# dylandreimerink/gobpfld

Measured on AMD Instinct MI355X. Metric: Mpkt/s device-resident XDP-emulator verdicts, 64B and 1500B batches, higher is better.
Workload: dtype int64

## Files before the change

### gobpfld_amd/csrc/xe_jit.cpp

```cpp
#ifndef XE_HOSTSIM
#include <hip/hip_runtime_api.h>
#include <hip/hiprtc.h>
#endif

#include <algorithm>
#include <array>
#include <atomic>
#include <chrono>
#include <climits>
#include <cstdint>
#include <cstdio>
#include <cstdlib>
#include <cstring>
#include <fstream>
#include <future>
#include <map>
#include <memory>
#include <set>
#include <mutex>
#include <sstream>
#include <string>
#include <vector>

#include <unistd.h>
// ... 1780 lines not shown
  if (buf && buflen) {
    const size_t c = s.size() < buflen - 1 ? s.size() : buflen - 1;
    memcpy(buf, s.data(), c);
    buf[c] = 0;
  }
  return s.size();
}

#ifndef XE_HOSTSIM
extern "C" int xe_jit_occupancy(void* fn, uint32_t nmaps) {
  int nb = 0;
  if (hipModuleOccupancyMaxActiveBlocksPerMultiprocessor(&nb, (hipFunction_t)fn, 256, (nmaps + 1) * sizeof(XeDevMap)) != hipSuccess) return 0;
  return nb;
}

extern "C" int xe_jit_launch(void* fn, const XeParams* P, uint32_t blocks, uint32_t threads, hipStream_t s) {
  XeParams p = *P;
  void* args[] = {&p};
  return hipModuleLaunchKernel((hipFunction_t)fn, blocks, 1, 1, threads, 1, 1, unsigned((p.nmaps + 1) * sizeof(XeDevMap)), s, args,
                               nullptr) == hipSuccess ? 0 : -1;
}

extern "C" int xe_jit_compile_check(const XeUop* prog, size_t n, char* buf, size_t buflen) {
  std::vector<XeUop> p(prog, prog + n);
  std::string err;
  std::vector<char> code = compile(generate_vm({std::vector<XeUop>(), p}, 1, demo_geom(), XE_JV_PLAIN, nullptr, nullptr), "gfx950", err);
  if (buf && buflen) {
    size_t c = err.size() < buflen - 1 ? err.size() : buflen - 1;
    memcpy(buf, err.data(), c);
    buf[c] = 0;
  }
  return code.empty() ? -1 : 0;
}

extern "C" int xe_jit_compile_check_keyed(const XeUop* prog, size_t n, char* buf, size_t buflen) {
// ... 47 lines not shown
```

### gobpfld_amd/csrc/xe_kernel.hip

```cpp
#include "xe_interp.h"
#include "xe_kernels.h"

#include <hipcub/device/device_radix_sort.hpp>
#include <hipcub/device/device_scan.hpp>

extern "C" __global__ void __launch_bounds__(256) xe_interp_kernel(XeParams P) {
  __shared__ __attribute__((aligned(16))) uint8_t hdr_lds[XE_HDR_LDS_BYTES];
  __shared__ XePend pend_lds[4];
  extern __shared__ __attribute__((aligned(16))) uint8_t xe_dyn_lds[];
  XeLane L;
  L.hdrbuf = (XE_LP(uint8_t))(hdr_lds + (threadIdx.x >> 6) * XE_HDR_WAVE_BYTES);
  const int lane = xe_lane();
  stage_maps(L, P, (XE_LP(XeDevMap))xe_dyn_lds);
  wave_state_init(L, P, (blockIdx.x * blockDim.x + threadIdx.x) >> 6, &pend_lds[threadIdx.x >> 6]);
  if (P.mode == XE_MODE_SEQUENTIAL) {
    if (blockIdx.x != 0 || threadIdx.x >= 64) return;
    seq_packets(L, P, [&](uint32_t i, bool valid) { run_staged(L, P, i, valid); }, [](bool) {});
  } else if (P.mode == XE_MODE_CHAIN) {
    chain_packets(L, P, blockIdx.x * blockDim.x + threadIdx.x, gridDim.x * blockDim.x,
                  [&](uint32_t i, bool valid) { run_staged(L, P, i, valid); });
  } else {
    const uint32_t wave = (blockIdx.x * blockDim.x + threadIdx.x) >> 6;
    const uint32_t nwaves = (gridDim.x * blockDim.x) >> 6;
    parallel_packets(L, P, wave, nwaves, [&](uint32_t i, bool valid) { run_staged(L, P, i, valid); });
// ... 49 lines not shown
  uint32_t nseg;
  unsigned long long* zero;
  uint64_t zero_words;
};
extern "C" __global__ void xe_prologue_kernel(XeProlog A) {
  const uint64_t tid = blockIdx.x * uint64_t(blockDim.x) + threadIdx.x, nth = uint64_t(gridDim.x) * blockDim.x;
  for (uint64_t i = tid; i < A.zero_words; i += nth) A.zero[i] = 0;
  for (uint32_t g = 0; g < A.nseg; g++)
    for (uint64_t i = tid; i < A.words[g]; i += nth) A.dst[g][i] = A.src[g][i];
}

extern "C" __global__ void __launch_bounds__(1024) xe_tail_kernel(XeTailArgs A) {
  __shared__ unsigned long long orw[257];
  const uint32_t t = threadIdx.x, nt = blockDim.x;
  for (uint32_t w = t; w <= 256; w += nt) orw[w] = 0;
  const bool poisoned = *(volatile uint32_t*)A.poison != 0;
  __syncthreads();
  for (uint32_t i = t; i < A.aux_words; i += nt) {
    const unsigned long long v = A.aux[i];
    if (v) A.aux[i] = 0;
    A.host_aux[i] = v;
    if (i == 0) orw[256] = v;
    else if (i >= 16 && v) atomicOr(&orw[(i - 16) % A.rep_words], v);
  }
  __syncthreads();
  if (t == 0) {
    const bool replay = !poisoned && xe_replay_decision(uint32_t(orw[256]), orw, A.rep_words, A.nmaps, A.mode);
    A.host_aux[XE_AUX_DECISION] = replay ? 1ull : 0ull;
    if (replay) *A.poison = 1u;
  }
  if (poisoned) return;
  for (uint32_t f = 0; f < A.ntail; f++) {
    const XeTailMap& T = A.tail[f];
    for (uint64_t i = t; i < T.words; i += nt) {
      unsigned long long r[16];
#pragma unroll
      for (uint32_t k = 0; k < 16; k++) r[k] = k < T.nrep ? T.rep[k * T.stride_words + i] : 0ull;
      unsigned long long s = 0;
#pragma unroll
      for (uint32_t k = 0; k < 16; k++) {
        s += r[k];
        if (r[k]) T.rep[k * T.stride_words + i] = 0;
      }
      const unsigned long long v = T.vals[i] + s;
      if (s) T.vals[i] = v;
      T.snap[i] = v;
    }
  }
}
extern "C" int xe_launch_tail(const XeTailArgs* A, hipStream_t s) {
  if (A->rep_words > 256) return -1;
  hipLaunchKernelGGL(xe_tail_kernel, dim3(1), dim3(1024), 0, s, *A);
  return hipGetLastError() == hipSuccess ? 0 : -1;
}

__global__ void xe_desc_split_kernel(const xe_desc* d, uint32_t n, uint64_t umem_len, unsigned long long* key,
                                     uint32_t* len) {
  for (uint64_t i = blockIdx.x * uint64_t(blockDim.x) + threadIdx.x; i < n; i += uint64_t(gridDim.x) * blockDim.x) {
    const uint64_t a = d[i].addr;
    uint32_t l = d[i].len;
    if (a > umem_len || uint64_t(l) > umem_len - a) l = 0;
    key[i] = l ? a : ~0ull;
    len[i] = l;
  }
}
__global__ void xe_desc_overlap_kernel(const unsigned long long* key, const uint32_t* len, uint32_t n, uint32_t* flag) {
  for (uint64_t i = blockIdx.x * uint64_t(blockDim.x) + threadIdx.x; i + 1 < n; i += uint64_t(gridDim.x) * blockDim.x)
// ... 232 lines not shown

extern "C" int xe_launch_keyed_esort(const XeKeyed* K, void* scratch, size_t* bytes, hipStream_t s) {
  size_t tmp = 0;
  if (hipcub::DeviceRadixSort::SortPairs(nullptr, tmp, (const unsigned long long*)nullptr, (unsigned long long*)nullptr,
                                         (const uint32_t*)nullptr, (uint32_t*)nullptr, int(K->dcap), 0, 64, s) != hipSuccess)
    return -1;
  if (!scratch) {
    *bytes = tmp;
    return 0;
  }
  if (*bytes < tmp) return -1;
  return hipcub::DeviceRadixSort::SortPairs(scratch, tmp, (const unsigned long long*)K->ekey, (unsigned long long*)K->ekey2,
                                            K->eval, K->eval2, int(K->dcap), 0, 64, s) == hipSuccess ? 0 : -1;
}

extern "C" int xe_launch_interp(const XeParams* P, uint32_t blocks, uint32_t threads, hipStream_t s) {
  hipLaunchKernelGGL(xe_interp_kernel, dim3(blocks), dim3(threads), (P->nmaps + 1) * sizeof(XeDevMap), s, *P);
  return hipGetLastError() == hipSuccess ? 0 : -1;
}
extern "C" int xe_interp_occupancy(uint32_t nmaps) {
  int nb = 0;
  if (hipOccupancyMaxActiveBlocksPerMultiprocessor(&nb, xe_interp_kernel, 256, (nmaps + 1) * sizeof(XeDevMap)) != hipSuccess) return 0;
  return nb;
}
template <class T, class C = T>
static int launch_delta_t(const void* cur, const void* snap, void* out, uint64_t n, hipStream_t s) {
  uint32_t blocks = uint32_t(n / 256 + 1);
  if (blocks > 4096) blocks = 4096;
  hipLaunchKernelGGL((xe_delta_kernel<T, C>), dim3(blocks), dim3(256), 0, s, (const T*)cur, (const T*)snap, (C*)out, n);
  return hipGetLastError() == hipSuccess ? 0 : -1;
}
template <class T, class C = T>
// ... 70 lines not shown
```

### gobpfld_amd/csrc/xe_kernels.h

```cpp
#ifndef XE_KERNELS_H_
#define XE_KERNELS_H_

#include "xe_internal.h"

#ifndef XE_HOSTSIM
#include <hip/hip_runtime_api.h>
#endif

extern "C" {

int xe_jit_may_write_entries(const XeUop* prog, size_t n);
size_t xe_jit_source_for(const XeUop* const* progs, const uint32_t* lens, uint32_t nprogs, int32_t entry,
                         const XeDevMap* maps, uint32_t nmaps, int variant, char* buf, size_t buflen);

#ifndef XE_HOSTSIM
void* xe_jit_get(const XeUop* const* progs, const uint32_t* lens, uint32_t nprogs, int32_t entry, int device,
                 const XeDevMap* maps, uint32_t nmaps, bool* cyclic, bool* general, const char** err, int variant,
                 uint64_t* maxpath);
int xe_jit_launch(void* fn, const XeParams* P, uint32_t blocks, uint32_t threads, hipStream_t s);
int xe_jit_occupancy(void* fn, uint32_t nmaps);

int xe_launch_interp(const XeParams* P, uint32_t blocks, uint32_t threads, hipStream_t s);
int xe_interp_occupancy(uint32_t nmaps);
int xe_launch_delta(const void* cur, const void* snap, void* out, uint64_t bytes, uint32_t lane, hipStream_t s);
int xe_launch_apply_delta(void* cur, const void* snap, const void* delta, uint64_t bytes, uint32_t lane, hipStream_t s);
int xe_launch_delta_sum(void* acc, const void* in, uint64_t bytes, uint32_t lane, hipStream_t s);
int xe_launch_rep_fold(void* vals, void* rep, uint64_t stride_words, uint32_t nrep, uint64_t nwords, const void* recs,
                       uint32_t rwords, uint32_t vsize, uint32_t cap, const void* lim, hipStream_t s);
int xe_launch_prologue(const void* const* src, void* const* dst, const uint64_t* words, uint32_t nseg, void* zero,
                       uint64_t zero_words, hipStream_t s);
int xe_launch_tail(const XeTailArgs* A, hipStream_t s);
int xe_launch_desc_overlap(const void* desc, uint32_t n, uint64_t umem_len, void* scratch, size_t* scratch_bytes,
                           uint32_t* flag, hipStream_t s);
int xe_launch_keyed(const XeKeyed* K, const XeDevMap* maps, uint8_t* skip, uint32_t step, uint32_t items, hipStream_t s);
int xe_launch_keyed_sort(const XeKeyed* K, uint32_t n, uint32_t end_bit, void* scratch, size_t* bytes, hipStream_t s);
int xe_launch_keyed_esort(const XeKeyed* K, void* scratch, size_t* bytes, hipStream_t s);
int xe_launch_keyed_scan(const XeKeyed* K, uint32_t n, void* scratch, size_t* bytes, hipStream_t s);
int xe_launch_append(const XeAppendArgs* A, uint32_t end_bit, void* scratch, size_t* bytes, hipStream_t s);
int xe_launch_pop(const uint32_t* src, uint32_t* dst, uint32_t n, uint32_t mode, uint32_t arg, XePopSlots sl, uint32_t* flag,
                  hipStream_t s);
int xe_launch_lru_relink(uint64_t* tag, uint32_t pool, uint32_t cnt, uint32_t* link, uint64_t* hdr, void* scratch,
                         size_t* bytes, int renumber, hipStream_t s);
int xe_launch_lru_tag_fold(uint64_t* tag, uint64_t* rep, uint32_t pool, uint32_t r, const uint64_t* hdr, hipStream_t s);
int xe_launch_lru_log(const uint64_t* tag, uint32_t pool, const uint32_t* order, const uint64_t* hdr, uint64_t* log,
                      hipStream_t s);
#endif
// ... 14 lines not shown
```

### gobpfld_amd/csrc/xe_runtime.cpp

```cpp
#include "xe_internal.h"
#include "xe_mapops.h"

#include <algorithm>
#include <map>
#include <chrono>
#include <cstdio>
#include <cstdlib>
#include <cstring>
#include <string>
#include <array>
#include <thread>
#include <vector>

#ifdef XE_HOSTSIM
#define XE_SEQ_PEEK 1
#include "xe_interp.h"
typedef void* xe_stream_t;
#else
#include <hip/hip_runtime_api.h>
typedef hipStream_t xe_stream_t;
#endif
#include "xe_kernels.h"

#define XE_FRAME_SIZE 256

namespace {

#ifdef XE_HOSTSIM
#ifdef XE_HOSTSIM_POISON
int dev_alloc(void** p, size_t n) {
  n = n ? n : 8;
  *p = malloc(n);
  if (*p) memset(*p, 0xA5, n);
  return *p ? 0 : -1;
}
#else
int dev_alloc(void** p, size_t n) { *p = calloc(n ? n : 8, 1); return *p ? 0 : -1; }
#endif
void dev_free(void* p) { free(p); }
int h2d(void* d, const void* h, size_t n, xe_stream_t) { memcpy(d, h, n); return 0; }
int d2h(void* h, const void* d, size_t n, xe_stream_t) { memcpy(h, d, n); return 0; }
int d2d(void* d, const void* s, size_t n, xe_stream_t) { memmove(d, s, n); return 0; }
int dmemset(void* d, int v, size_t n, xe_stream_t) { memset(d, v, n); return 0; }
int dsync(xe_stream_t) { return 0; }
int launch_interp(const XeParams* P, uint32_t, uint32_t, xe_stream_t) {
  XeLane L;
#ifdef XE_HOSTSIM_POISON
  memset(static_cast<void*>(&L), 0, sizeof L);
#endif
  static thread_local uint8_t hdrbuf[XE_HDR_WAVE_BYTES + 16];
  L.hdrbuf = hdrbuf;
  XePend pend;
  stage_maps(L, *P, nullptr);
  wave_state_init(L, *P, 0, &pend);
  if (P->mode == XE_MODE_PARALLEL || P->mode == XE_MODE_SPEC) {
    parallel_packets(L, *P, 0, 1, [&](uint32_t i, bool valid) { run_staged(L, *P, i, valid); });
  } else if (P->mode == XE_MODE_CHAIN) {
    chain_packets(L, *P, 0, 1, [&](uint32_t i, bool valid) { run_staged(L, *P, i, valid); });
  } else {
    seq_packets(L, *P, [&](uint32_t i, bool valid) { run_staged(L, *P, i, valid); },
                [&](bool valid) { run_staged(L, *P, 0, valid, false); });
  }
  flush_wave_state(L, *P);
  return 0;
}
int launch_jit(void*, const XeParams* P, uint32_t b, uint32_t t, xe_stream_t s) { return launch_interp(P, b, t, s); }
template <class T, class C = T>
void lanes_sub(const void* a, const void* b, void* o, uint64_t n) {
  for (uint64_t i = 0; i < n; i++) ((C*)o)[i] = C(T(((const T*)a)[i] - ((const T*)b)[i]));
}
template <class T, class C = T>
void lanes_add(const void* snap, const void* d, void* o, uint64_t n) {
  for (uint64_t i = 0; i < n; i++) ((T*)o)[i] = T(((const T*)snap)[i] + T(((const C*)d)[i]));
}
template <class C>
void lanes_acc(void* acc, const void* in, uint64_t n) {
  for (uint64_t i = 0; i < n; i++) ((C*)acc)[i] = C(((C*)acc)[i] + ((const C*)in)[i]);
}
int launch_delta(const void* cur, const void* snap, void* out, uint64_t bytes, uint32_t lane, xe_stream_t) {
  switch (lane) {
    case 1: lanes_sub<uint8_t>(cur, snap, out, bytes); break;
// ... 29 lines not shown
int launch_rep_fold(void* vals, void* rep, uint64_t sw, uint32_t nrep, uint64_t nw, const void* recs, uint32_t rwords,
                    uint32_t vsize, uint32_t cap, const void* lim, xe_stream_t) {
  uint64_t* v = (uint64_t*)vals;
  uint64_t* r = (uint64_t*)rep;
  const uint64_t* rc = (const uint64_t*)recs;
  if (lim) nw = std::min<uint64_t>(nw, (((const uint64_t*)lim)[3] * vsize + 7) / 8);
  for (uint64_t i = 0; i < nw; i++) {
    if (rc) {
      const uint64_t s0 = 8 * i / vsize, s1 = (8 * i + 7) / vsize;
      if (!((s0 <= cap && rc[s0 * rwords]) || (s1 != s0 && s1 <= cap && rc[s1 * rwords]))) continue;
    }
    for (uint32_t k = 0; k < nrep; k++) { v[i] += r[k * sw + i]; r[k * sw + i] = 0; }
  }
  return 0;
}
int launch_tail(const XeTailArgs* A, xe_stream_t) {
  unsigned long long orw[257] = {};
  const bool poisoned = *A->poison != 0;
  for (uint32_t i = 0; i < A->aux_words; i++) {
    const unsigned long long v = A->aux[i];
    A->aux[i] = 0;
    A->host_aux[i] = v;
    if (i == 0) orw[256] = v;
    else if (i >= 16) orw[(i - 16) % A->rep_words] |= v;
  }
  const bool replay = !poisoned && xe_replay_decision(uint32_t(orw[256]), orw, A->rep_words, A->nmaps, A->mode);
  A->host_aux[XE_AUX_DECISION] = replay ? 1ull : 0ull;
  if (replay) *A->poison = 1u;
  if (poisoned) return 0;
  for (uint32_t f = 0; f < A->ntail; f++) {
    const XeTailMap& T = A->tail[f];
    for (uint64_t i = 0; i < T.words; i++) {
      unsigned long long s = 0;
      for (uint32_t k = 0; k < T.nrep; k++) { s += T.rep[k * T.stride_words + i]; T.rep[k * T.stride_words + i] = 0; }
      T.vals[i] += s;
      T.snap[i] = T.vals[i];
    }
  }
  return 0;
}
// ... 118 lines not shown
  if (A->perf) rec.assign(A->rec + 2 * A->base, A->rec + 2 * (A->base + A->k));
  for (uint32_t j = 0; j < A->k; j++) {
    const uint32_t id = v[j].second;
    if (A->perf) {
      A->rec[2 * (A->base + j)] = rec[2 * (id - A->base)];
      A->rec[2 * (A->base + j) + 1] = rec[2 * (id - A->base) + 1];
    } else {
      A->link[A->stack ? A->cnt0 + j : (A->head + A->cnt0 + j) % A->list_cap] = id;
    }
  }
  return 0;
}
struct Timer {
  std::chrono::steady_clock::time_point t;
  void rec(xe_stream_t) { t = std::chrono::steady_clock::now(); }
  static float ms(const Timer& a, const Timer& b) { return std::chrono::duration<float, std::milli>(b.t - a.t).count(); }
  int wait() { return 0; }
  void init() {}
  void fini() {}
};
int set_device(int) { return 0; }
int blocks_per_cu(void*, uint32_t) { return 1; }
int cu_count(int) { return 1; }
#else
int dev_alloc(void** p, size_t n) { return hipMalloc(p, n ? n : 8) == hipSuccess ? 0 : -1; }
void dev_free(void* p) { if (p) (void)hipFree(p); }
int h2d(void* d, const void* h, size_t n, xe_stream_t s) { return hipMemcpyAsync(d, h, n, hipMemcpyHostToDevice, s) == hipSuccess ? 0 : -1; }
int d2h(void* h, const void* d, size_t n, xe_stream_t s) { return hipMemcpyAsync(h, d, n, hipMemcpyDeviceToHost, s) == hipSuccess ? 0 : -1; }
int d2d(void* d, const void* src, size_t n, xe_stream_t s) { return hipMemcpyAsync(d, src, n, hipMemcpyDeviceToDevice, s) == hipSuccess ? 0 : -1; }
int dmemset(void* d, int v, size_t n, xe_stream_t s) { return hipMemsetAsync(d, v, n, s) == hipSuccess ? 0 : -1; }
int dsync(xe_stream_t s) { return hipStreamSynchronize(s) == hipSuccess ? 0 : -1; }
int launch_interp(const XeParams* P, uint32_t b, uint32_t t, xe_stream_t s) { return xe_launch_interp(P, b, t, s); }
int launch_jit(void* fn, const XeParams* P, uint32_t b, uint32_t t, xe_stream_t s) { return xe_jit_launch(fn, P, b, t, s); }
int launch_delta(const void* c, const void* sn, void* o, uint64_t b, uint32_t lane, xe_stream_t s) {
  return xe_launch_delta(c, sn, o, b, lane, s);
}
int launch_apply_delta(void* c, const void* sn, const void* d, uint64_t b, uint32_t lane, xe_stream_t s) {
  return xe_launch_apply_delta(c, sn, d, b, lane, s);
}
int launch_rep_fold(void* v, void* r, uint64_t sw, uint32_t nrep, uint64_t nw, const void* recs, uint32_t rwords, uint32_t vsize,
                    uint32_t cap, const void* lim, xe_stream_t s) {
  return xe_launch_rep_fold(v, r, sw, nrep, nw, recs, rwords, vsize, cap, lim, s);
}
int launch_delta_sum(void* acc, const void* in, uint64_t bytes, uint32_t lane, xe_stream_t s) {
  return xe_launch_delta_sum(acc, in, bytes, lane, s);
}
int launch_prologue(const void* const* src, void* const* dst, const uint64_t* words, uint32_t nseg, void* zero, uint64_t zw,
                    xe_stream_t s) {
// ... 18 lines not shown
}
int launch_keyed_scan(const XeKeyed* K, uint32_t n, void* scratch, size_t* bytes, xe_stream_t s) {
  return xe_launch_keyed_scan(K, n, scratch, bytes, s);
}
void host_free(void* p) { if (p) (void)hipHostFree(p); }
int launch_lru_relink(uint64_t* tag, uint32_t pool, uint32_t cnt, uint32_t* link, uint64_t* hdr, void* scratch,
                      size_t* bytes, int renumber, xe_stream_t s) {
  return xe_launch_lru_relink(tag, pool, cnt, link, hdr, scratch, bytes, renumber, s);
}
int launch_lru_tag_fold(uint64_t* tag, uint64_t* rep, uint32_t pool, uint32_t r, const uint64_t* hdr, xe_stream_t s) {
  return xe_launch_lru_tag_fold(tag, rep, pool, r, hdr, s);
}
int launch_lru_log(const uint64_t* tag, uint32_t pool, const uint32_t* order, const uint64_t* hdr, uint64_t* log, xe_stream_t s) {
  return xe_launch_lru_log(tag, pool, order, hdr, log, s);
}
int launch_tail(const XeTailArgs* A, xe_stream_t s) { return xe_launch_tail(A, s); }
int launch_desc_overlap(const void* desc, uint32_t n, uint64_t umem_len, void* scratch, size_t* bytes, uint32_t* flag,
                        xe_stream_t s) {
  return xe_launch_desc_overlap(desc, n, umem_len, scratch, bytes, flag, s);
}
int host_device_ptr(void** d, void* h) { return hipHostGetDevicePointer(d, h, 0) == hipSuccess ? 0 : -1; }
int host_alloc_coherent(void** p, size_t n) {
  if (hipHostMalloc(p, n ? n : 8, hipHostMallocCoherent | hipHostMallocMapped) != hipSuccess) return -1;
  memset(*p, 0, n);
  return 0;
}
int serve_hostcalls(XeHostCall* H, xe_stream_t s) {
  for (;;) {
    const uint32_t req = __atomic_load_n(&H->req, __ATOMIC_ACQUIRE);
    if (req != __atomic_load_n(&H->ack, __ATOMIC_RELAXED)) {
      const uint32_t id = H->id;
// ... 12 lines not shown
    if (q != hipErrorNotReady) return -1;
    std::this_thread::sleep_for(std::chrono::microseconds(20));
  }
}
int poison_async(uint32_t* d, xe_stream_t* cs) {
  if (!*cs && hipStreamCreateWithFlags(cs, hipStreamNonBlocking) != hipSuccess) return -1;
  if (hipMemsetD32Async(reinterpret_cast<hipDeviceptr_t>(d), 2u, 1, *cs) != hipSuccess) return -1;
  return hipStreamSynchronize(*cs) == hipSuccess ? 0 : -1;
}
void stream_destroy(xe_stream_t s) { if (s) (void)hipStreamDestroy(s); }
struct Timer {
  hipEvent_t e = nullptr;
  void init() { if (!e) (void)hipEventCreate(&e); }
  void fini() { if (e) (void)hipEventDestroy(e); e = nullptr; }
  void rec(xe_stream_t s) { init(); (void)hipEventRecord(e, s); }
  int wait() { return hipEventSynchronize(e) == hipSuccess ? 0 : -1; }
  static float ms(const Timer& a, const Timer& b) { float m = 0; (void)hipEventElapsedTime(&m, a.e, b.e); return m; }
};
int set_device(int d) { return hipSetDevice(d) == hipSuccess ? 0 : -1; }
int blocks_per_cu(void* jit, uint32_t nmaps) { return jit ? xe_jit_occupancy(jit, nmaps) : xe_interp_occupancy(nmaps); }
int cu_count(int dev) {
  int n = 0;
  if (hipDeviceGetAttribute(&n, hipDeviceAttributeMultiprocessorCount, dev) != hipSuccess) return 0;
  return n;
}
#endif
int launch_emulator(void* fn, const XeParams* P, uint32_t blocks, uint32_t threads, xe_stream_t s) {
  return fn ? launch_jit(fn, P, blocks, threads, s) : launch_interp(P, blocks, threads, s);
}

int size_log2(uint8_t sizecode) {
  switch (sizecode) { case 0x00: return 2; case 0x08: return 1; case 0x10: return 0; default: return 3; }
}

XeUop fail_uop(int code) { XeUop u{}; u.cls = U_FAIL; u.imm = code; return u; }

int translate(const uint64_t* raw, uint32_t n, std::vector<XeUop>& out, std::string& err) {
  out.assign(n, XeUop{});
  for (uint32_t i = 0; i < n; i++) {
    const uint64_t r = raw[i];
    const uint8_t op = uint8_t(r);
    const uint8_t dst = uint8_t(r >> 8) & 0x0f, src = uint8_t(r >> 12) & 0x0f;
    const int16_t off = int16_t(uint16_t(r >> 16));
// ... 391 lines not shown
    bool ready = false;
    void* fn = nullptr;
  };
  std::array<Variant, 4> jit_variants{};
  Timer t0, t1, t2;
  uint64_t ord_slack = 4096, ord_slack_bytes = 1 << 20;
  struct Batch {
    void* d_umem = nullptr; uint64_t umem_len = 0; const void* d_desc = nullptr; uint32_t n = 0;
    void* d_results = nullptr; void* d_verdicts = nullptr; void* d_regs = nullptr;
    xe_stream_t s = nullptr; xe_batch_stats* stats = nullptr;
  };
  struct Slot {
    unsigned long long* d_aux = nullptr;
    unsigned long long* h_aux = nullptr;
    unsigned long long* h_aux_dev = nullptr;
    Timer t0, t1, done;
    Batch b;
    size_t aux_used = 0;
    uint32_t nmaps = 0, grid = 0, engine = 0;
    uint32_t snap = 0;
  };
  std::array<Slot, kAsyncDepth> slots;
  std::vector<uint32_t> pending;
  uint32_t next_slot = 0;
  uint32_t next_snap = 0;
  uint32_t* d_poison = nullptr;
  xe_stream_t cancel_stream = nullptr;
  int32_t staged_slot = -1;
  bool draining = false;
  bool delta_base = true;
  bool epoch_open = false;
// ... 690 lines not shown
  if (vm->settings.stack_frame_size != 256 || vm->settings.max_stack_frames != 8) {
    delete vm;
    return XE_ERR_UNSUPPORTED;
  }
  if (set_device(vm->settings.device)) { delete vm; return XE_ERR_DEVICE; }
#ifndef XE_HOSTSIM
  if (hipStreamCreateWithFlags(&vm->stream, hipStreamNonBlocking) != hipSuccess) { delete vm; return XE_ERR_DEVICE; }
#endif
  *out = vm;
  return XE_OK;
}

void xe_destroy(xe_vm* vm) {
  if (!vm) return;
  set_device(vm->settings.device);
  for (uint32_t si : vm->pending) (void)vm->slots[si].done.wait();
  vm->pending.clear();
  for (auto& sl : vm->slots) {
    dev_free(sl.d_aux); host_free(sl.h_aux);
    sl.t0.fini(); sl.t1.fini(); sl.done.fini();
  }
  dev_free(vm->d_poison);
  stream_destroy(vm->cancel_stream);
  dev_free(vm->d_trace_pk); dev_free(vm->d_trace); dev_free(vm->d_trace_cnt);
  dev_free(vm->d_listrun); dev_free(vm->d_popflag); dev_free(vm->d_popbase); dev_free(vm->d_popused);
  host_free(vm->h_hostcall);
  for (auto& m : vm->maps) map_free_device(m);
  dev_free(vm->d_progs); dev_free(vm->d_prog_off); dev_free(vm->d_maps); dev_free(vm->d_aux);
  dev_free(vm->d_arena_par); dev_free(vm->d_arena_seq); dev_free(vm->d_ksnap);
  dev_free(vm->d_umem); dev_free(vm->d_desc); dev_free(vm->d_res); dev_free(vm->d_ver); dev_free(vm->d_regs);
  dev_free(vm->d_usnap); dev_free(vm->d_ovl); dev_free(vm->d_app); dev_free(vm->d_app_sort); dev_free(vm->d_relink);
  dev_free(vm->d_mo); dev_free(vm->d_mo_keys); dev_free(vm->d_mo_vals); dev_free(vm->d_mo_found); dev_free(vm->d_mo_join); dev_free(vm->d_ms);
  keyed_free(vm);
  vm->t0.fini(); vm->t1.fini(); vm->t2.fini();
#ifndef XE_HOSTSIM
// ... 716 lines not shown
  return g;
}

void reduce_aux(const unsigned long long* aux, uint32_t nmaps, uint32_t rep_words, std::vector<unsigned long long>& red) {
  red.assign(16 + 2 * size_t(nmaps + 1), 0);
  red[0] = aux[0];
  for (uint32_t r = 0; r < kRep; r++) {
    const unsigned long long* rec = aux + 16 + size_t(r) * rep_words;
    red[1] += rec[0];
    for (int k = 0; k < 8; k++) red[2 + k] += rec[1 + k];
    for (int k = 0; k < 4; k++) red[XE_REC_WIDTH0 + 2 + k] |= rec[XE_REC_WIDTH0 + k];
    for (uint32_t w = 0; w < 2 * (nmaps + 1); w++) red[16 + w] |= rec[16 + w];
  }
}

bool run_conflict(const std::vector<unsigned long long>& red, uint32_t nmaps) {
  bool conflict = (uint32_t(red[0]) & (XE_FLAG_ORDERED | XE_FLAG_CAPACITY)) != 0;
  for (uint32_t m = 1; m <= nmaps && m < 64; m++) {
    if (red[16 + 2 * m] & red[16 + 2 * m + 1]) conflict = true;
    const unsigned wc = unsigned(red[XE_REC_WIDTH0 + 2 + m / 16] >> (4 * (m % 16))) & 15u;
    if (wc & (wc - 1)) conflict = true;
  }
  return conflict;
}

uint32_t lane_of(unsigned wc) { return wc == 0u ? 0u : wc == 1u ? 1u : wc == 2u ? 2u : wc == 4u ? 4u : 8u; }

void record_widths(xe_vm* vm, const std::vector<unsigned long long>& red, uint32_t nmaps) {
  for (uint32_t m = 1; m <= nmaps && m < 64; m++) {
    const unsigned wc = unsigned(red[XE_REC_WIDTH0 + 2 + m / 16] >> (4 * (m % 16))) & 15u;
// ... 320 lines not shown
  }
  for (int attempt = 0;; attempt++) {
    P.mode = XE_MODE_SEQUENTIAL;
    if (general && ensure_arena(vm, true, 1, P.gen)) return fail(vm, XE_ERR_NOMEM, "device alloc (replay arena)");
    bool table = false;
    for (size_t i = 1; i < vm->maps.size(); i++) {
      if (vm->maps[i].dkind != XE_DM_LRU) continue;
      const int r = lru_log_build(vm, vm->maps[i], s);
      if (r < 0) return fail(vm, XE_ERR_DEVICE, "LRU order log");
      table = table || r > 0;
    }
    if (table) {
      if (int rc = upload_map_table(vm, s)) return rc;
      P.maps = vm->d_maps;
    }
    vm->t1.rec(s);
    void* sj = (jit && !jit_general && n >= kSeqScalarMin) ? variant_kernel(vm, jit, kSeqVariant) : nullptr;
    if (launch_emulator(sj ? sj : jit, &P, 1, 64, s)) return fail(vm, XE_ERR_DEVICE, "kernel launch");
    vm->t2.rec(s);
    if (hostcalls && serve_hostcalls(vm->h_hostcall, s)) return fail(vm, XE_ERR_DEVICE, "kernel failed (host helpers)");
    if (read_aux()) return fail(vm, XE_ERR_DEVICE, "kernel failed");
    kms += Timer::ms(vm->t1, vm->t2);
    if (!(red[0] & XE_FLAG_CAPACITY)) {
      for (size_t i = 1; i < vm->maps.size(); i++)
        if (vm->maps[i].dkind == XE_DM_LRU) vm->maps[i].links_stale = true;
      return XE_OK;
    }
    if (attempt >= 6) return fail(vm, XE_ERR_NOMEM, "the ordered replay outgrew its device arena");
    vm->seq_scale *= 4;
    vm->ord_slack *= 4;
    vm->ord_slack_bytes *= 4;
    if (rollback(true)) return fail(vm, XE_ERR_DEVICE, "rollback");
    for (size_t i = 1; i < vm->maps.size(); i++) {
      HostMap& m = vm->maps[i];
// ... 304 lines not shown
      return fail(vm, XE_ERR_NOMEM, "device alloc (pop ranks)");
    vm->pop_n = n;
  }
  return XE_OK;
}

int BatchRun::list_init() {
  memset(&lr, 0, sizeof lr);
  for (size_t i = 1; i < vm->maps.size() && i < 64; i++)
    if (vm->maps[i].dkind == XE_DM_LIST) lr.cnt0[i] = uint32_t(ord_h0[i * 8 + 1]);
  for (int i = 0; i < 64; i++) lr.push[i] = lr.senslo[i] = 0xffffffffu;
  return h2d(vm->d_listrun, &lr, sizeof lr, s);
}

int BatchRun::pass() {
  if (launch_emulator(pj, &P, vm->last_grid, 256, s)) return fail(vm, XE_ERR_DEVICE, "kernel launch");
  vm->t1.rec(s);
  if (fold()) return fail(vm, XE_ERR_DEVICE, "replica fold");
  if (read_aux()) return fail(vm, XE_ERR_DEVICE, "kernel failed");
  kms = Timer::ms(vm->t0, vm->t1);
  flags = uint32_t(red[0]);
  conflict = run_conflict(red, P.nmaps);
  return XE_OK;
}

int BatchRun::ranked_passes() {
  P.pop_mode = 1;
  P.popflag = vm->d_popflag;
  P.popbase = nullptr;
  if (dmemset(vm->d_popflag, 0, size_t(n) * 4, s)) return fail(vm, XE_ERR_DEVICE, "pop flags");
  if (int rc = pass()) return rc;
  tmark("count pass");
// ... 208 lines not shown
    rc = b.keyed_first();
  } else {
    if ((rc = b.parallel())) return rc;
    if (b.conflict && automatic && b.seg_cut >= kSegMin && b.seg_cut < n && segments_ok(vm, b.P)) {
      if (b.rollback(false) || (b.ordmaps && ordered_hdr_restore(vm, b.ord_h0, b.s))) return fail(vm, XE_ERR_DEVICE, "rollback");
      return run_segments(vm, d_umem, umem_len, d_desc, n, b.seg_cut, d_results, d_verdicts, d_regs, stream, stats);
    }
    if (b.conflict && (automatic || (b.flags & XE_FLAG_CAPACITY))) rc = b.after_conflict();
    else if (!b.conflict) rc = b.results_stand();
  }
  return rc ? rc : b.publish();
}

namespace {

int complete_oldest(xe_vm* vm) {
  const uint32_t si = vm->pending.front();
  xe_vm::Slot& sl = vm->slots[si];
  if (sl.done.wait()) {
    vm->pending.clear();
    return fail(vm, XE_ERR_DEVICE, "kernel failed (pipelined batch)");
  }
  const unsigned long long* aux = sl.h_aux;
  if (aux[XE_AUX_DECISION]) {
    vm->staged_slot = -1;
    const xe_stream_t s = sl.b.s;
    for (size_t i = 1; i < vm->maps.size(); i++) {
      HostMap& m = vm->maps[i];
      if (!m.ordered() && d2d(m.d_vals, m.d_asnap[sl.snap], m.vals_alloc, s)) return fail(vm, XE_ERR_DEVICE, "rollback");
    }
    if (dmemset(vm->d_poison, 0, 4, s)) return fail(vm, XE_ERR_DEVICE, "rollback");
    std::vector<xe_vm::Batch> redo;
    for (uint32_t k : vm->pending) redo.push_back(vm->slots[k].b);
    vm->pending.clear();
    for (const xe_vm::Batch& b : redo)
      if (int rc = xe_run_batch_device(vm, b.d_umem, b.umem_len, b.d_desc, b.n, b.d_results, b.d_verdicts, b.d_regs, b.s,
                                       b.stats))
        return rc;
    return XE_OK;
  }
  std::vector<unsigned long long> red;
  reduce_aux(aux, sl.nmaps, 16 + 2 * (sl.nmaps + 1), red);
  record_widths(vm, red, sl.nmaps);
  note_run(vm, red, XE_MODE_PARALLEL);
  if (sl.b.stats)
    publish_stats(sl.b.stats, red, sl.b.n, XE_MODE_PARALLEL, run_conflict(red, sl.nmaps), Timer::ms(sl.t0, sl.t1), sl.engine,
                  sl.grid);
  vm->pending.erase(vm->pending.begin());
  return XE_OK;
}

}

int xe_prepare(xe_vm* vm) {
  if (!vm) return XE_ERR_INVAL;
  if (int rc = xe_sync(vm)) return rc;
  if (int rc = prepare_run(vm, vm->stream)) return rc;
  void* jit = nullptr;
  bool jit_general = false;
  if (int rc = select_engine(vm, jit, jit_general)) return rc;
  if (jit && keyed_candidate(vm)) variant_kernel(vm, jit, kKeyedVariant);
// ... 167 lines not shown
    }
  if (int rc = prepare_run(vm, s)) return rc;
  void* jit = nullptr;
  bool jit_general = false;
  if (int rc = select_engine(vm, jit, jit_general)) return rc;
  const bool general = !jit || jit_general;

  const uint32_t si = vm->next_slot;
  const uint32_t ai = vm->next_snap, nai = (ai + 1) % (kAsyncDepth + 1);
  xe_vm::Slot& sl = vm->slots[si];
  if (!sl.d_aux) {
    if (dev_alloc((void**)&sl.d_aux, kAuxWords * 8) || dmemset(sl.d_aux, 0, kAuxWords * 8, s))
      return fail(vm, XE_ERR_DEVICE, "alloc (pipelined batch records)");
  }
  if (!sl.h_aux) {
    if (host_alloc((void**)&sl.h_aux, kAuxWords * 8) || host_device_ptr((void**)&sl.h_aux_dev, sl.h_aux))
      return fail(vm, XE_ERR_DEVICE, "alloc (pipelined batch records)");
  }
  if (!vm->d_poison) {
    if (dev_alloc((void**)&vm->d_poison, 8) || dmemset(vm->d_poison, 0, 8, s)) return fail(vm, XE_ERR_DEVICE, "alloc (poison)");
  }
  XeParams P = batch_params(vm, d_umem, umem_len, d_desc, n, d_results, d_verdicts, d_regs, sl.d_aux);
  P.mode = XE_MODE_PARALLEL;
  P.poison = vm->d_poison;
  const size_t aux_used = 16 + size_t(kRep) * P.rep_words;
  const bool staged = vm->staged_slot == int32_t(ai) && !vm->pending.empty() && vm->slots[vm->pending.back()].b.s == s;
  XeTailArgs A{};
  A.aux = sl.d_aux;
  A.host_aux = sl.h_aux_dev;
  A.poison = vm->d_poison;
  A.aux_words = uint32_t(aux_used);
// ... 21 lines not shown
      T.nrep = m.nrep > 1 ? m.nrep : 0;
    } else {
      big.push_back(i);
    }
    if (!small || !staged) {
      src.push_back(m.d_vals);
      dst.push_back(m.d_asnap[ai]);
      words.push_back(m.vals_alloc / 8);
    }
  }
  if (jit && !P.results && !P.regs) jit = variant_kernel(vm, jit, kLeanVariant);
  const uint32_t grid = parallel_grid(vm, jit, general, n, P.nmaps);
  if (general && ensure_arena(vm, false, grid * 256, P.gen)) return fail(vm, XE_ERR_NOMEM, "device alloc (arena)");
  if (!src.empty() && launch_prologue(src.data(), dst.data(), words.data(), uint32_t(src.size()), nullptr, 0, s))
    return fail(vm, XE_ERR_DEVICE, "prologue");
  sl.t0.rec(s);
  if (launch_emulator(jit, &P, grid, 256, s)) return fail(vm, XE_ERR_DEVICE, "kernel launch");
  sl.t1.rec(s);
  for (size_t i : big) {
    HostMap& m = vm->maps[i];
    if (m.nrep > 1 && fold_map(m, s))
      return fail(vm, XE_ERR_DEVICE, "replica fold");
  }
  if (launch_tail(&A, s)) return fail(vm, XE_ERR_DEVICE, "epilogue");
  sl.done.rec(s);
  vm->staged_slot = int32_t(nai);
  sl.snap = ai;
  vm->next_snap = nai;
  sl.b = xe_vm::Batch{d_umem, umem_len, d_desc, n, d_results, d_verdicts, d_regs, s, stats};
  sl.aux_used = aux_used;
  sl.nmaps = P.nmaps;
  sl.grid = grid;
  sl.engine = jit ? XE_ENGINE_JIT : XE_ENGINE_INTERP;
  vm->last_grid = grid;
  vm->pending.push_back(si);
  vm->next_slot = (si + 1) % kAsyncDepth;
  vm->delta_base = false;
  for (size_t i = 1; i < vm->maps.size(); i++) vm->maps[i].dev_dirty = true;
  return XE_OK;
}
// ... 1104 lines not shown
```

Before: 60820.

## Fold timing events into kernel launches and reduce aux records on device

Replaces separate hipEventRecord calls around the emulator and tail kernels with hipExtLaunchKernel start/stop events, and reuses the previous batch's done event as the start marker when batches are chained. The tail kernel now reduces the per-replica aux record on device (sums for count fields, OR for flags) and writes only the reduced record to host memory, which is now allocated coherent, so the host skips reduce_aux. It also prefetches the first tail map's replica words before the poison check. This cuts per-batch stream marker commands and the size of host-visible writes, at the cost of more complex event bookkeeping with double-buffered done events. The old marker path remains available behind an env flag.

```diff
diff --git a/gobpfld_amd/csrc/xe_jit.cpp b/gobpfld_amd/csrc/xe_jit.cpp
--- a/gobpfld_amd/csrc/xe_jit.cpp
+++ b/gobpfld_amd/csrc/xe_jit.cpp
@@ -1,5 +1,6 @@
 #ifndef XE_HOSTSIM
 #include <hip/hip_runtime_api.h>
+#include <hip/hip_ext.h>
 #include <hip/hiprtc.h>
 #endif
 
@@ -1818,11 +1819,16 @@
   return nb;
 }
 
-extern "C" int xe_jit_launch(void* fn, const XeParams* P, uint32_t blocks, uint32_t threads, hipStream_t s) {
+extern "C" int xe_jit_launch(void* fn, const XeParams* P, uint32_t blocks, uint32_t threads, hipStream_t s, hipEvent_t start,
+                             hipEvent_t stop) {
   XeParams p = *P;
   void* args[] = {&p};
-  return hipModuleLaunchKernel((hipFunction_t)fn, blocks, 1, 1, threads, 1, 1, unsigned((p.nmaps + 1) * sizeof(XeDevMap)), s, args,
-                               nullptr) == hipSuccess ? 0 : -1;
+  const unsigned lds = unsigned((p.nmaps + 1) * sizeof(XeDevMap));
+  if (!start && !stop)
+    return hipModuleLaunchKernel((hipFunction_t)fn, blocks, 1, 1, threads, 1, 1, lds, s, args, nullptr) == hipSuccess ? 0 : -1;
+  if (uint64_t(blocks) * threads > 0xffffffffull) return -1;
+  return hipExtModuleLaunchKernel((hipFunction_t)fn, blocks * threads, 1, 1, threads, 1, 1, lds, s, args, nullptr, start, stop, 0) ==
+                 hipSuccess ? 0 : -1;
 }
 
 extern "C" int xe_jit_compile_check(const XeUop* prog, size_t n, char* buf, size_t buflen) {
diff --git a/gobpfld_amd/csrc/xe_kernel.hip b/gobpfld_amd/csrc/xe_kernel.hip
--- a/gobpfld_amd/csrc/xe_kernel.hip
+++ b/gobpfld_amd/csrc/xe_kernel.hip
@@ -1,6 +1,7 @@
 #include "xe_interp.h"
 #include "xe_kernels.h"
 
+#include <hip/hip_ext.h>
 #include <hipcub/device/device_radix_sort.hpp>
 #include <hipcub/device/device_scan.hpp>
 
@@ -87,43 +88,54 @@
   __shared__ unsigned long long orw[257];
   const uint32_t t = threadIdx.x, nt = blockDim.x;
   for (uint32_t w = t; w <= 256; w += nt) orw[w] = 0;
+  unsigned long long pr[16], pv = 0;
+  const bool pre = A.ntail && t < A.tail[0].words;
+#pragma unroll
+  for (uint32_t k = 0; k < 16; k++) pr[k] = pre && k < A.tail[0].nrep ? A.tail[0].rep[k * A.tail[0].stride_words + t] : 0ull;
+  if (pre) pv = A.tail[0].vals[t];
   const bool poisoned = *(volatile uint32_t*)A.poison != 0;
   __syncthreads();
   for (uint32_t i = t; i < A.aux_words; i += nt) {
     const unsigned long long v = A.aux[i];
     if (v) A.aux[i] = 0;
-    A.host_aux[i] = v;
+    if (i < 16) A.host_aux[i] = v;
     if (i == 0) orw[256] = v;
-    else if (i >= 16 && v) atomicOr(&orw[(i - 16) % A.rep_words], v);
+    else if (i >= 16 && v) {
+      const uint32_t w = (i - 16) % A.rep_words;
+      if (w < XE_REC_WIDTH0) atomicAdd(&orw[w], v);
+      else atomicOr(&orw[w], v);
+    }
   }
   __syncthreads();
+  for (uint32_t w = t; w < A.rep_words; w += nt) A.host_aux[16 + w] = orw[w];
   if (t == 0) {
     const bool replay = !poisoned && xe_replay_decision(uint32_t(orw[256]), orw, A.rep_words, A.nmaps, A.mode);
     A.host_aux[XE_AUX_DECISION] = replay ? 1ull : 0ull;
     if (replay) *A.poison = 1u;
   }
-  if (poisoned) return;
-  for (uint32_t f = 0; f < A.ntail; f++) {
+  for (uint32_t f = 0; f < (poisoned ? 0u : A.ntail); f++) {
     const XeTailMap& T = A.tail[f];
     for (uint64_t i = t; i < T.words; i += nt) {
+      const bool ahead = f == 0 && i == t;
       unsigned long long r[16];
 #pragma unroll
-      for (uint32_t k = 0; k < 16; k++) r[k] = k < T.nrep ? T.rep[k * T.stride_words + i] : 0ull;
+      for (uint32_t k = 0; k < 16; k++) r[k] = ahead ? pr[k] : k < T.nrep ? T.rep[k * T.stride_words + i] : 0ull;
       unsigned long long s = 0;
 #pragma unroll
       for (uint32_t k = 0; k < 16; k++) {
         s += r[k];
         if (r[k]) T.rep[k * T.stride_words + i] = 0;
       }
-      const unsigned long long v = T.vals[i] + s;
+      const unsigned long long v = (ahead ? pv : T.vals[i]) + s;
       if (s) T.vals[i] = v;
       T.snap[i] = v;
     }
   }
 }
-extern "C" int xe_launch_tail(const XeTailArgs* A, hipStream_t s) {
+extern "C" int xe_launch_tail(const XeTailArgs* A, hipStream_t s, hipEvent_t start, hipEvent_t stop) {
   if (A->rep_words > 256) return -1;
-  hipLaunchKernelGGL(xe_tail_kernel, dim3(1), dim3(1024), 0, s, *A);
+  if (start || stop) hipExtLaunchKernelGGL(xe_tail_kernel, dim3(1), dim3(1024), 0, s, start, stop, 0, *A);
+  else hipLaunchKernelGGL(xe_tail_kernel, dim3(1), dim3(1024), 0, s, *A);
   return hipGetLastError() == hipSuccess ? 0 : -1;
 }
 
@@ -386,8 +398,11 @@
                                             K->eval, K->eval2, int(K->dcap), 0, 64, s) == hipSuccess ? 0 : -1;
 }
 
-extern "C" int xe_launch_interp(const XeParams* P, uint32_t blocks, uint32_t threads, hipStream_t s) {
-  hipLaunchKernelGGL(xe_interp_kernel, dim3(blocks), dim3(threads), (P->nmaps + 1) * sizeof(XeDevMap), s, *P);
+extern "C" int xe_launch_interp(const XeParams* P, uint32_t blocks, uint32_t threads, hipStream_t s, hipEvent_t start,
+                                hipEvent_t stop) {
+  const uint32_t lds = (P->nmaps + 1) * sizeof(XeDevMap);
+  if (start || stop) hipExtLaunchKernelGGL(xe_interp_kernel, dim3(blocks), dim3(threads), lds, s, start, stop, 0, *P);
+  else hipLaunchKernelGGL(xe_interp_kernel, dim3(blocks), dim3(threads), lds, s, *P);
   return hipGetLastError() == hipSuccess ? 0 : -1;
 }
 extern "C" int xe_interp_occupancy(uint32_t nmaps) {
diff --git a/gobpfld_amd/csrc/xe_kernels.h b/gobpfld_amd/csrc/xe_kernels.h
--- a/gobpfld_amd/csrc/xe_kernels.h
+++ b/gobpfld_amd/csrc/xe_kernels.h
@@ -17,10 +17,11 @@
 void* xe_jit_get(const XeUop* const* progs, const uint32_t* lens, uint32_t nprogs, int32_t entry, int device,
                  const XeDevMap* maps, uint32_t nmaps, bool* cyclic, bool* general, const char** err, int variant,
                  uint64_t* maxpath);
-int xe_jit_launch(void* fn, const XeParams* P, uint32_t blocks, uint32_t threads, hipStream_t s);
+int xe_jit_launch(void* fn, const XeParams* P, uint32_t blocks, uint32_t threads, hipStream_t s, hipEvent_t start,
+                  hipEvent_t stop);
 int xe_jit_occupancy(void* fn, uint32_t nmaps);
 
-int xe_launch_interp(const XeParams* P, uint32_t blocks, uint32_t threads, hipStream_t s);
+int xe_launch_interp(const XeParams* P, uint32_t blocks, uint32_t threads, hipStream_t s, hipEvent_t start, hipEvent_t stop);
 int xe_interp_occupancy(uint32_t nmaps);
 int xe_launch_delta(const void* cur, const void* snap, void* out, uint64_t bytes, uint32_t lane, hipStream_t s);
 int xe_launch_apply_delta(void* cur, const void* snap, const void* delta, uint64_t bytes, uint32_t lane, hipStream_t s);
@@ -29,7 +30,7 @@
                        uint32_t rwords, uint32_t vsize, uint32_t cap, const void* lim, hipStream_t s);
 int xe_launch_prologue(const void* const* src, void* const* dst, const uint64_t* words, uint32_t nseg, void* zero,
                        uint64_t zero_words, hipStream_t s);
-int xe_launch_tail(const XeTailArgs* A, hipStream_t s);
+int xe_launch_tail(const XeTailArgs* A, hipStream_t s, hipEvent_t start, hipEvent_t stop);
 int xe_launch_desc_overlap(const void* desc, uint32_t n, uint64_t umem_len, void* scratch, size_t* scratch_bytes,
                            uint32_t* flag, hipStream_t s);
 int xe_launch_keyed(const XeKeyed* K, const XeDevMap* maps, uint8_t* skip, uint32_t step, uint32_t items, hipStream_t s);
diff --git a/gobpfld_amd/csrc/xe_runtime.cpp b/gobpfld_amd/csrc/xe_runtime.cpp
--- a/gobpfld_amd/csrc/xe_runtime.cpp
+++ b/gobpfld_amd/csrc/xe_runtime.cpp
@@ -16,9 +16,11 @@
 #define XE_SEQ_PEEK 1
 #include "xe_interp.h"
 typedef void* xe_stream_t;
+typedef std::chrono::steady_clock::time_point* xe_event_t;
 #else
 #include <hip/hip_runtime_api.h>
 typedef hipStream_t xe_stream_t;
+typedef hipEvent_t xe_event_t;
 #endif
 #include "xe_kernels.h"
 
@@ -43,7 +45,9 @@
 int d2d(void* d, const void* s, size_t n, xe_stream_t) { memmove(d, s, n); return 0; }
 int dmemset(void* d, int v, size_t n, xe_stream_t) { memset(d, v, n); return 0; }
 int dsync(xe_stream_t) { return 0; }
-int launch_interp(const XeParams* P, uint32_t, uint32_t, xe_stream_t) {
+void stamp(xe_event_t e) { if (e) *e = std::chrono::steady_clock::now(); }
+int launch_interp(const XeParams* P, uint32_t, uint32_t, xe_stream_t, xe_event_t start, xe_event_t stop) {
+  stamp(start);
   XeLane L;
 #ifdef XE_HOSTSIM_POISON
   memset(static_cast<void*>(&L), 0, sizeof L);
@@ -62,9 +66,12 @@
                 [&](bool valid) { run_staged(L, *P, 0, valid, false); });
   }
   flush_wave_state(L, *P);
+  stamp(stop);
   return 0;
 }
-int launch_jit(void*, const XeParams* P, uint32_t b, uint32_t t, xe_stream_t s) { return launch_interp(P, b, t, s); }
+int launch_jit(void*, const XeParams* P, uint32_t b, uint32_t t, xe_stream_t s, xe_event_t start, xe_event_t stop) {
+  return launch_interp(P, b, t, s, start, stop);
+}
 template <class T, class C = T>
 void lanes_sub(const void* a, const void* b, void* o, uint64_t n) {
   for (uint64_t i = 0; i < n; i++) ((C*)o)[i] = C(T(((const T*)a)[i] - ((const T*)b)[i]));
@@ -124,16 +131,20 @@
   }
   return 0;
 }
-int launch_tail(const XeTailArgs* A, xe_stream_t) {
+int launch_tail(const XeTailArgs* A, xe_stream_t, xe_event_t start, xe_event_t stop) {
+  stamp(start);
   unsigned long long orw[257] = {};
   const bool poisoned = *A->poison != 0;
   for (uint32_t i = 0; i < A->aux_words; i++) {
     const unsigned long long v = A->aux[i];
     A->aux[i] = 0;
-    A->host_aux[i] = v;
+    if (i < 16) A->host_aux[i] = v;
     if (i == 0) orw[256] = v;
+    else if (i >= 16 && (i - 16) % A->rep_words < XE_REC_WIDTH0) orw[(i - 16) % A->rep_words] += v;
     else if (i >= 16) orw[(i - 16) % A->rep_words] |= v;
   }
+  for (uint32_t w = 0; w < A->rep_words; w++) A->host_aux[16 + w] = orw[w];
+  stamp(stop);
   const bool replay = !poisoned && xe_replay_decision(uint32_t(orw[256]), orw, A->rep_words, A->nmaps, A->mode);
   A->host_aux[XE_AUX_DECISION] = replay ? 1ull : 0ull;
   if (replay) *A->poison = 1u;
@@ -282,6 +293,8 @@
 struct Timer {
   std::chrono::steady_clock::time_point t;
   void rec(xe_stream_t) { t = std::chrono::steady_clock::now(); }
+  xe_event_t bind() { return &t; }
+  bool busy() { return false; }
   static float ms(const Timer& a, const Timer& b) { return std::chrono::duration<float, std::milli>(b.t - a.t).count(); }
   int wait() { return 0; }
   void init() {}
@@ -298,8 +311,12 @@
 int d2d(void* d, const void* src, size_t n, xe_stream_t s) { return hipMemcpyAsync(d, src, n, hipMemcpyDeviceToDevice, s) == hipSuccess ? 0 : -1; }
 int dmemset(void* d, int v, size_t n, xe_stream_t s) { return hipMemsetAsync(d, v, n, s) == hipSuccess ? 0 : -1; }
 int dsync(xe_stream_t s) { return hipStreamSynchronize(s) == hipSuccess ? 0 : -1; }
-int launch_interp(const XeParams* P, uint32_t b, uint32_t t, xe_stream_t s) { return xe_launch_interp(P, b, t, s); }
-int launch_jit(void* fn, const XeParams* P, uint32_t b, uint32_t t, xe_stream_t s) { return xe_jit_launch(fn, P, b, t, s); }
+int launch_interp(const XeParams* P, uint32_t b, uint32_t t, xe_stream_t s, xe_event_t start, xe_event_t stop) {
+  return xe_launch_interp(P, b, t, s, start, stop);
+}
+int launch_jit(void* fn, const XeParams* P, uint32_t b, uint32_t t, xe_stream_t s, xe_event_t start, xe_event_t stop) {
+  return xe_jit_launch(fn, P, b, t, s, start, stop);
+}
 int launch_delta(const void* c, const void* sn, void* o, uint64_t b, uint32_t lane, xe_stream_t s) {
   return xe_launch_delta(c, sn, o, b, lane, s);
 }
@@ -348,7 +365,7 @@
 int launch_lru_log(const uint64_t* tag, uint32_t pool, const uint32_t* order, const uint64_t* hdr, uint64_t* log, xe_stream_t s) {
   return xe_launch_lru_log(tag, pool, order, hdr, log, s);
 }
-int launch_tail(const XeTailArgs* A, xe_stream_t s) { return xe_launch_tail(A, s); }
+int launch_tail(const XeTailArgs* A, xe_stream_t s, xe_event_t start, xe_event_t stop) { return xe_launch_tail(A, s, start, stop); }
 int launch_desc_overlap(const void* desc, uint32_t n, uint64_t umem_len, void* scratch, size_t* bytes, uint32_t* flag,
                         xe_stream_t s) {
   return xe_launch_desc_overlap(desc, n, umem_len, scratch, bytes, flag, s);
@@ -391,6 +408,8 @@
   void init() { if (!e) (void)hipEventCreate(&e); }
   void fini() { if (e) (void)hipEventDestroy(e); e = nullptr; }
   void rec(xe_stream_t s) { init(); (void)hipEventRecord(e, s); }
+  xe_event_t bind() { init(); return e; }
+  bool busy() { return e && hipEventQuery(e) == hipErrorNotReady; }
   int wait() { return hipEventSynchronize(e) == hipSuccess ? 0 : -1; }
   static float ms(const Timer& a, const Timer& b) { float m = 0; (void)hipEventElapsedTime(&m, a.e, b.e); return m; }
 };
@@ -402,8 +421,10 @@
   return n;
 }
 #endif
-int launch_emulator(void* fn, const XeParams* P, uint32_t blocks, uint32_t threads, xe_stream_t s) {
-  return fn ? launch_jit(fn, P, blocks, threads, s) : launch_interp(P, blocks, threads, s);
+int launch_emulator(void* fn, const XeParams* P, uint32_t blocks, uint32_t threads, xe_stream_t s, Timer* start = nullptr,
+                    Timer* stop = nullptr) {
+  const xe_event_t a = start ? start->bind() : nullptr, b = stop ? stop->bind() : nullptr;
+  return fn ? launch_jit(fn, P, blocks, threads, s, a, b) : launch_interp(P, blocks, threads, s, a, b);
 }
 
 int size_log2(uint8_t sizecode) {
@@ -825,7 +846,9 @@
     unsigned long long* d_aux = nullptr;
     unsigned long long* h_aux = nullptr;
     unsigned long long* h_aux_dev = nullptr;
-    Timer t0, t1, done;
+    Timer t0, t1, done[2];
+    uint32_t turn = 0;
+    Timer* from = nullptr;
     Batch b;
     size_t aux_used = 0;
     uint32_t nmaps = 0, grid = 0, engine = 0;
@@ -1546,11 +1569,11 @@
 void xe_destroy(xe_vm* vm) {
   if (!vm) return;
   set_device(vm->settings.device);
-  for (uint32_t si : vm->pending) (void)vm->slots[si].done.wait();
+  for (uint32_t si : vm->pending) (void)vm->slots[si].done[vm->slots[si].turn].wait();
   vm->pending.clear();
   for (auto& sl : vm->slots) {
     dev_free(sl.d_aux); host_free(sl.h_aux);
-    sl.t0.fini(); sl.t1.fini(); sl.done.fini();
+    sl.t0.fini(); sl.t1.fini(); sl.done[0].fini(); sl.done[1].fini();
   }
   dev_free(vm->d_poison);
   stream_destroy(vm->cancel_stream);
@@ -2297,6 +2320,16 @@
   }
 }
 
+void reduced_record(const unsigned long long* aux, uint32_t nmaps, std::vector<unsigned long long>& red) {
+  red.assign(16 + 2 * size_t(nmaps + 1), 0);
+  const unsigned long long* rec = aux + 16;
+  red[0] = aux[0];
+  red[1] = rec[0];
+  for (int k = 0; k < 8; k++) red[2 + k] = rec[1 + k];
+  for (int k = 0; k < 4; k++) red[XE_REC_WIDTH0 + 2 + k] = rec[XE_REC_WIDTH0 + k];
+  for (uint32_t w = 0; w < 2 * (nmaps + 1); w++) red[16 + w] = rec[16 + w];
+}
+
 bool run_conflict(const std::vector<unsigned long long>& red, uint32_t nmaps) {
   bool conflict = (uint32_t(red[0]) & (XE_FLAG_ORDERED | XE_FLAG_CAPACITY)) != 0;
   for (uint32_t m = 1; m <= nmaps && m < 64; m++) {
@@ -2647,10 +2680,8 @@
       if (int rc = upload_map_table(vm, s)) return rc;
       P.maps = vm->d_maps;
     }
-    vm->t1.rec(s);
     void* sj = (jit && !jit_general && n >= kSeqScalarMin) ? variant_kernel(vm, jit, kSeqVariant) : nullptr;
-    if (launch_emulator(sj ? sj : jit, &P, 1, 64, s)) return fail(vm, XE_ERR_DEVICE, "kernel launch");
-    vm->t2.rec(s);
+    if (launch_emulator(sj ? sj : jit, &P, 1, 64, s, &vm->t1, &vm->t2)) return fail(vm, XE_ERR_DEVICE, "kernel launch");
     if (hostcalls && serve_hostcalls(vm->h_hostcall, s)) return fail(vm, XE_ERR_DEVICE, "kernel failed (host helpers)");
     if (read_aux()) return fail(vm, XE_ERR_DEVICE, "kernel failed");
     kms += Timer::ms(vm->t1, vm->t2);
@@ -2985,8 +3016,7 @@
 }
 
 int BatchRun::pass() {
-  if (launch_emulator(pj, &P, vm->last_grid, 256, s)) return fail(vm, XE_ERR_DEVICE, "kernel launch");
-  vm->t1.rec(s);
+  if (launch_emulator(pj, &P, vm->last_grid, 256, s, &vm->t0, &vm->t1)) return fail(vm, XE_ERR_DEVICE, "kernel launch");
   if (fold()) return fail(vm, XE_ERR_DEVICE, "replica fold");
   if (read_aux()) return fail(vm, XE_ERR_DEVICE, "kernel failed");
   kms = Timer::ms(vm->t0, vm->t1);
@@ -3225,10 +3255,15 @@
 
 namespace {
 
+bool markers3() {
+  static const bool on = xe_tuning_env("XE_MARKERS3") != nullptr;
+  return on;
+}
+
 int complete_oldest(xe_vm* vm) {
   const uint32_t si = vm->pending.front();
   xe_vm::Slot& sl = vm->slots[si];
-  if (sl.done.wait()) {
+  if (sl.done[sl.turn].wait()) {
     vm->pending.clear();
     return fail(vm, XE_ERR_DEVICE, "kernel failed (pipelined batch)");
   }
@@ -3251,11 +3286,11 @@
     return XE_OK;
   }
   std::vector<unsigned long long> red;
-  reduce_aux(aux, sl.nmaps, 16 + 2 * (sl.nmaps + 1), red);
+  reduced_record(aux, sl.nmaps, red);
   record_widths(vm, red, sl.nmaps);
   note_run(vm, red, XE_MODE_PARALLEL);
   if (sl.b.stats)
-    publish_stats(sl.b.stats, red, sl.b.n, XE_MODE_PARALLEL, run_conflict(red, sl.nmaps), Timer::ms(sl.t0, sl.t1), sl.engine,
+    publish_stats(sl.b.stats, red, sl.b.n, XE_MODE_PARALLEL, run_conflict(red, sl.nmaps), Timer::ms(*sl.from, sl.t1), sl.engine,
                   sl.grid);
   vm->pending.erase(vm->pending.begin());
   return XE_OK;
@@ -3453,7 +3488,7 @@
       return fail(vm, XE_ERR_DEVICE, "alloc (pipelined batch records)");
   }
   if (!sl.h_aux) {
-    if (host_alloc((void**)&sl.h_aux, kAuxWords * 8) || host_device_ptr((void**)&sl.h_aux_dev, sl.h_aux))
+    if (host_alloc_coherent((void**)&sl.h_aux, kAuxWords * 8) || host_device_ptr((void**)&sl.h_aux_dev, sl.h_aux))
       return fail(vm, XE_ERR_DEVICE, "alloc (pipelined batch records)");
   }
   if (!vm->d_poison) {
@@ -3505,16 +3540,21 @@
   if (general && ensure_arena(vm, false, grid * 256, P.gen)) return fail(vm, XE_ERR_NOMEM, "device alloc (arena)");
   if (!src.empty() && launch_prologue(src.data(), dst.data(), words.data(), uint32_t(src.size()), nullptr, 0, s))
     return fail(vm, XE_ERR_DEVICE, "prologue");
-  sl.t0.rec(s);
-  if (launch_emulator(jit, &P, grid, 256, s)) return fail(vm, XE_ERR_DEVICE, "kernel launch");
-  sl.t1.rec(s);
+  Timer* before = staged && src.empty() && !markers3() ? &vm->slots[vm->pending.back()].done[vm->slots[vm->pending.back()].turn] : nullptr;
+  const bool chained = before && before->busy();
+  sl.turn ^= 1;
+  sl.from = chained ? before : &sl.t0;
+  if (markers3()) sl.t0.rec(s);
+  if (launch_emulator(jit, &P, grid, 256, s, chained || markers3() ? nullptr : &sl.t0, markers3() ? nullptr : &sl.t1))
+    return fail(vm, XE_ERR_DEVICE, "kernel launch");
+  if (markers3()) sl.t1.rec(s);
   for (size_t i : big) {
     HostMap& m = vm->maps[i];
     if (m.nrep > 1 && fold_map(m, s))
       return fail(vm, XE_ERR_DEVICE, "replica fold");
   }
-  if (launch_tail(&A, s)) return fail(vm, XE_ERR_DEVICE, "epilogue");
-  sl.done.rec(s);
+  if (launch_tail(&A, s, nullptr, markers3() ? nullptr : sl.done[sl.turn].bind())) return fail(vm, XE_ERR_DEVICE, "epilogue");
+  if (markers3()) sl.done[sl.turn].rec(s);
   vm->staged_slot = int32_t(nai);
   sl.snap = ai;
   vm->next_snap = nai;
```

Result: faster. 63320, median of 6 (+4.1%).
